# maxsonate/video-diffusion-nnx

Hardware: AMD Instinct MI355X
Metric: denoised frames/sec, 16fx64x64 1000-step DDPM (higher is better)
Workload: dtype bf16; 1 GPU; config_v2_2 (north-star shape): Unet3D dim=64 C=1, 16f x 64x64, DDPM T=1000 p_sample_loop (UNet forward + p_sample per step, hipGraph replay); value = n_gpus*B*F/(T*s_per_step); batch_per_gpu=64, parallelism=dp1 (independent samples, no collective), mfma_operands=bf16, storage=weights fp32 master, activations bf16, fp32 accumulate, process_group=none (single process)

## Files before the change

### video_diffusion_nnx_amd/csrc/conv_ws.hip

```cpp
#include "vdx_common.h"
#include "vdx_internal.h"
#include "vdx_glds.h"
#include <type_traits>

namespace vdx {

namespace {

__device__ __attribute__((aligned(16))) unsigned g_zero_page[4];

__device__ __forceinline__ int frag_off(int row, int key, int q) { return row * 128 + (((q ^ (key & 3)) | (key & 4)) << 4); }

constexpr int WS_SLAB = 128 * 128;
constexpr int WS_STORES = 16;

}

constexpr int WS_NS = 4;

template <int GEO> struct WsGeo {
    static constexpr bool WF = GEO != 0;
    static constexpr int S = WF ? GEO : 16;
    static constexpr int NP = WF ? 256 / (S * S) : 1;
    static constexpr int IW = 18;
    static constexpr int HPX = WF ? 257 : 18 * 18;
    static constexpr int NPIECE = HPX * 8;
    static constexpr int NU = (NPIECE + 511) / 512;
    static constexpr int NUMIN = NPIECE / 512;
    static constexpr int HBUF = HPX * 128;
};

template <int GEO, bool PRO>
__global__ __launch_bounds__(512, 2) void conv3x3_ws_kernel(const ConvArgs P, const int tiles_per_range, const int total_tiles, const int nct, const int pin) {
    using M = Mma<MODE_BF16>;
    using G = WsGeo<GEO>;
    constexpr bool WF = G::WF;
    constexpr int S = G::S, NP = G::NP, IW = G::IW, HPX = G::HPX, NPIECE = G::NPIECE, NU = G::NU, NUMIN = G::NUMIN, HBUF = G::HBUF;
    constexpr int NS = WS_NS;
    constexpr int WIN = 2;

    extern __shared__ __attribute__((aligned(16))) char smem[];
    char* ring = smem;
    char* halo = ring + NS * WS_SLAB;
    float* biasl = reinterpret_cast<float*>(halo + 2 * HBUF);
    float* coefA = biasl + 128;
    float* coefD = coefA + P.CinPad;
    float* gmean = coefD + P.CinPad;

    const unsigned ring_a = lds_addr(ring), halo_a = lds_addr(halo);
    const int tid = threadIdx.x, lane = tid & 63;
    const int wave = __builtin_amdgcn_readfirstlane(tid >> 6);
    const int r = lane & 15, q = lane >> 4;
    const int wc = wave & 1, wpx = wave >> 1;
    const int xcd = blockIdx.x & 7, slot = blockIdx.x >> 3;
    const int j = pin ? xcd % nct : slot % nct;
    const int range = pin ? slot * (8 / nct) + xcd / nct : (slot / nct) * 8 + xcd;
    const int t0 = range * tiles_per_range, t1 = min(t0 + tiles_per_range, total_tiles);
    if (t0 >= t1) return;
    const int tiles_x = WF ? 1 : P.W / 16, tiles_pf = WF ? 1 : tiles_x * (P.H / 16);
    const int nchunks = P.CinPad >> 6;
    const int Cin = P.C0 + P.C1;
    const int fpt = NP;
    const int tps = WF ? (P.F + NP - 1) / NP : 1;
    auto sample_of = [&](int t) { return WF ? t / tps : (t / tiles_pf) / P.F; };
    auto wf_pix0 = [&](int t) { const int b = t / tps, k = t - b * tps; return (unsigned)(b * P.F + k * NP) * (unsigned)(S * S); };
    auto wf_rows = [&](int t) { const int k = t % tps; return min(NP, P.F - k * NP) * (S * S); };

    unsigned wsrc[2];
#pragma unroll
    for (int v = 0; v < 2; ++v) {
        const int i2 = (v * 8 + wave) * 64 + lane, row = i2 >> 3, pos = i2 & 7;
        wsrc[v] = (unsigned)((j * 128 + row) * P.CinPad) * 2u + (unsigned)((pos ^ (row & 7)) << 4);
    }
    const size_t tap_stride = (size_t)P.Cout * P.CinPad * 2;
    const char* wbase = reinterpret_cast<const char*>(P.wp);
    auto piece = [&](int u, int l, int& row, int& chunk) -> bool {
        const int i = (u * 8 + wave) * 64 + l;
        row = i >> 3;
        const int key = WF ? row : row - ((row * 3641) >> 16) * IW;
        chunk = (i & 7) ^ (key & 7);
        return i < NPIECE;
    };
    auto opaque_lane = [&]() { int l = lane; asm volatile("" : "+v"(l)); return l; };
    const char* const zero_page = reinterpret_cast<const char*>(g_zero_page);
    constexpr int DYB = (WF ? S : IW) * 128;
    const int halo_o = NS * WS_SLAB;
    const int aoff = frag_off(wc * 64 + r, r, q);
    int b3[4][3], zs[3];
    int opix[4];
#pragma unroll
    for (int tn = 0; tn < 4; ++tn) {
        if (!WF) {
            const int py = wpx * 4 + tn, px = r;
            opix[tn] = py * P.W + px;
#pragma unroll
            for (int dx = 0; dx < 3; ++dx) b3[tn][dx] = halo_o + frag_off(py * IW + px + dx, px + dx, q);
        } else {
            const int p = wpx * 64 + tn * 16 + r;
            opix[tn] = p;
#pragma unroll
            for (int dx = 0; dx < 3; ++dx) b3[tn][dx] = halo_o + frag_off(p - S - 1 + dx, p - 1 + dx, q);
        }
    }
#pragma unroll
    for (int dy = 0; dy < 3; ++dy) zs[dy] = halo_o + 256 * 128 + (q << 4) - dy * DYB;
    auto tap_valid = [&](int tn, int dy, int dx) -> bool {
        const int p = wpx * 64 + tn * 16 + r, y = (p / S) % S + dy - 1, x = p % S + dx - 1;
        return y >= 0 && y < S && x >= 0 && x < S;
    };
    if (tid < 128) biasl[tid] = P.bias ? P.bias[j * 128 + tid] : 0.f;

    int pcc = 0, ptap = 0, pslot = 0;
    auto issue_w = [&]() {
        const char* src = wbase + (size_t)ptap * tap_stride + (size_t)(pcc << 7);
        const unsigned dst = __builtin_amdgcn_readfirstlane(ring_a + pslot * WS_SLAB + wave * 1024);
        glds16(src + wsrc[0], dst);
        glds16(src + wsrc[1], dst + 8 * 1024);
        if (++ptap == 9) { ptap = 0; if (++pcc == nchunks) pcc = 0; }
        if (++pslot == NS) pslot = 0;
    };
    unsigned okmask = 0;
    auto issue_halo = [&](int t, int cc, int buf) {
        const bool second = (cc << 6) >= P.C0;
        const char* xb = reinterpret_cast<const char*>(second ? P.x1 : P.x0);
        const int Cs = second ? P.C1 : P.C0, cb = (cc << 6) - (second ? P.C0 : 0);
        const unsigned dst = __builtin_amdgcn_readfirstlane(halo_a + buf * HBUF + wave * 1024);
        okmask = 0;
        const int l = opaque_lane();
        if (WF) {
            const unsigned pix0 = wf_pix0(t);
            const int nrows = wf_rows(t);
#pragma unroll
            for (int u = 0; u < NU; ++u) {
                int row, ch;
                if (piece(u, l, row, ch)) {
                    const bool ok = row < nrows;
                    const unsigned off = ((pix0 + row) * Cs + cb + (ch << 3)) * 2u;
                    const void* src = ok ? static_cast<const void*>(xb + off) : static_cast<const void*>(zero_page);
                    glds16(src, dst + u * 8 * 1024);
                    okmask |= ok ? (1u << u) : 0u;
                }
            }
        } else {
            const int f = t / tiles_pf, rem = t - f * tiles_pf, ty = rem / tiles_x, tx = rem - ty * tiles_x;
#pragma unroll
            for (int u = 0; u < NU; ++u) {
                int row, ch;
                if (piece(u, l, row, ch)) {
                    const int iy = (row * 3641) >> 16, ix = row - iy * IW;
                    const int gy = ty * 16 - 1 + iy, gx = tx * 16 - 1 + ix;
                    const bool ok = gy >= 0 && gy < P.H && gx >= 0 && gx < P.W;
                    const unsigned off = ((unsigned)((f * P.H + gy) * P.W + gx) * Cs + cb + (ch << 3)) * 2u;
                    const void* src = ok ? static_cast<const void*>(xb + off) : static_cast<const void*>(zero_page);
                    glds16(src, dst + u * 8 * 1024);
                    okmask |= ok ? (1u << u) : 0u;
                }
            }
        }
    };
    auto transform = [&](int u, int cc, int buf) {
        int row, ch;
        const int l = opaque_lane();
        if (!piece(u, l, row, ch) || !((okmask >> u) & 1u)) return;
        char* p = halo + buf * HBUF + ((u * 8 + wave) * 64 + l) * 16;
        const int c = (cc << 6) + (ch << 3);
#pragma unroll
        for (int h = 0; h < 2; ++h) {
            const uint2 v = *reinterpret_cast<const uint2*>(p + 8 * h);
            const float4 a = *reinterpret_cast<const float4*>(coefA + c + 4 * h);
            const float4 d = *reinterpret_cast<const float4*>(coefD + c + 4 * h);
            uint2 o;
            o.x = pack_bf16x2(silu_f(fmaf(__uint_as_float(v.x << 16), a.x, d.x)), silu_f(fmaf(__uint_as_float(v.x & 0xFFFF0000u), a.y, d.y)));
            o.y = pack_bf16x2(silu_f(fmaf(__uint_as_float(v.y << 16), a.z, d.z)), silu_f(fmaf(__uint_as_float(v.y & 0xFFFF0000u), a.w, d.w)));
            *reinterpret_cast<uint2*>(p + 8 * h) = o;
            asm volatile("" ::: "memory");
        }
    };
    auto make_coef = [&](int b) {
        gn_mean_rstd_wg(P.in_stats, b, P.groups, (double)P.F * P.H * P.W * (Cin / P.groups), gmean, tid, 512);
        __syncthreads();
        const int cpg = Cin / P.groups;
        for (int c = tid; c < Cin; c += 512) {
            const int g = c / cpg;
            const float m = gmean[2 * g], rs = gmean[2 * g + 1];
            const float ga = P.gamma[c], be = P.beta[c];
            float sc = 1.f, sh = 0.f;
            if (P.ss) { sc = P.ss[(size_t)b * P.ss_stride + c] + 1.f; sh = P.ss[(size_t)b * P.ss_stride + Cin + c]; }
            coefA[c] = rs * ga * sc;
            coefD[c] = (be - m * rs * ga) * sc + sh;
        }
        __syncthreads();
    };
    float st_s[4] = {0.f, 0.f, 0.f, 0.f}, st_q[4] = {0.f, 0.f, 0.f, 0.f};
    auto flush_stats = [&](int b) {
        if (!P.out_stats) return;
        const int cpg = P.Cout / P.out_groups;
#pragma unroll
        for (int tm = 0; tm < 4; ++tm) {
            const float s1 = reduce_q(reduce16(st_s[tm])), s2 = reduce_q(reduce16(st_q[tm]));
            st_s[tm] = 0.f; st_q[tm] = 0.f;
            if (lane == 0) {
                const int g = (j * 128 + wc * 64 + tm * 16) / cpg;
                double* dst = P.out_stats + (((size_t)b * GN_SLOTS + ((blockIdx.x + wave) % GN_SLOTS)) * P.out_groups + g) * 2;
                unsafeAtomicAdd(dst, (double)s1); unsafeAtomicAdd(dst + 1, (double)s2);
            }
        }
    };
    auto ldA1 = [&](int sl, int tm, int ks) -> uint4 {
        return *reinterpret_cast<const uint4*>(ring + sl * WS_SLAB + ((aoff + tm * 2048) ^ (ks * 64)));
    };
    auto ldB = [&](uint4 (&b)[4], int tap, int ks) {
        const int dy = tap / 3, dx = tap - 3 * dy;
#pragma unroll
        for (int tn = 0; tn < 4; ++tn) {
            int a = b3[tn][dx];
            if (WF) a = tap_valid(tn, dy, dx) ? a : zs[dy];
            b[tn] = *reinterpret_cast<const uint4*>(smem + ((a ^ (ks * 64)) + dy * DYB));
        }
    };
    auto flip_buffers = [&](int to_buf1) {
        const int d = to_buf1 ? HBUF : -HBUF;
#pragma unroll
        for (int tn = 0; tn < 4; ++tn)
#pragma unroll
            for (int dx = 0; dx < 3; ++dx) b3[tn][dx] += d;
#pragma unroll
        for (int dy = 0; dy < 3; ++dy) zs[dy] += d;
    };

    int bcoef = -1;
    const int b0 = sample_of(t0);
    if (PRO) { make_coef(b0); bcoef = b0; }
    issue_halo(t0, 0, 0);
#pragma unroll
    for (int k = 0; k < NS - 1; ++k) issue_w();
    wait_vm_lgkm0<0>();
    __builtin_amdgcn_s_barrier();
    if (PRO) {
#pragma unroll
        for (int u = 0; u < NU; ++u) transform(u, 0, 0);
        wait_vm_lgkm0<0>();
        __builtin_amdgcn_s_barrier();
    }

    int cslot = 0, hbuf = 0, bcur = b0;
    f32x4 acc[4][4];
    uint4 pb[4], pa;
    ldB(pb, 0, 0); pa = ldA1(0, 0, 0);
    auto run_chunk = [&](auto after_epi, int tnext, int ccnext, bool xform) {
        constexpr int EPI = decltype(after_epi)::value ? WS_STORES : 0;
#pragma unroll
        for (int tap = 0; tap < 9; ++tap) {
            if (tap == 0) wait_vm<WIN + EPI>();
            else if (tap == 1) wait_vm<WIN + NUMIN + EPI>();
            else wait_vm<WIN>();
            __builtin_amdgcn_s_barrier();
            if (tap == 0) issue_halo(tnext, ccnext, hbuf ^ 1);
            issue_w();
            const bool do_x = PRO && xform && tap >= 2 && tap - 2 < NU;
            if (do_x && wave < 4) {
                transform(tap - 2, ccnext, hbuf ^ 1);
                if (NU > 6 && tap == 7) transform(6, ccnext, hbuf ^ 1);
            }
#pragma unroll
            for (int tm = 0; tm < 4; ++tm) {
                const uint4 a = tm == 0 ? pa : ldA1(cslot, tm, 0);
#pragma unroll
                for (int tn = 0; tn < 4; ++tn) M::mma(acc[tm][tn], a, pb[tn]);
            }
            if (do_x && wave >= 4) {
                transform(tap - 2, ccnext, hbuf ^ 1);
                if (NU > 6 && tap == 7) transform(6, ccnext, hbuf ^ 1);
            }
            {
                uint4 b1[4];
                ldB(b1, tap, 1);
#pragma unroll
                for (int tm = 0; tm < 4; ++tm) {
                    const uint4 a = ldA1(cslot, tm, 1);
#pragma unroll
                    for (int tn = 0; tn < 4; ++tn) M::mma(acc[tm][tn], a, b1[tn]);
                }
            }
            const int nslot = (cslot + 1 == NS) ? 0 : cslot + 1;
            if (tap == 8) flip_buffers(hbuf ^ 1);
            ldB(pb, tap == 8 ? 0 : tap + 1, 0);
            pa = ldA1(nslot, 0, 0);
            cslot = nslot;
        }
        hbuf ^= 1;
    };

    bool after_epilogue = false;
    for (int t = t0; t < t1; ++t) {
#pragma unroll
        for (int tm = 0; tm < 4; ++tm)
#pragma unroll
            for (int tn = 0; tn < 4; ++tn) acc[tm][tn] = f32x4{0.f, 0.f, 0.f, 0.f};
        for (int cc = 0; cc < nchunks; ++cc) {
            const bool last = (cc + 1 == nchunks);
            const bool more = !last || (t + 1 < t1);
            const int tnext = last ? (t + 1 < t1 ? t + 1 : t) : t, ccnext = last ? 0 : cc + 1;
            if (PRO && more) {
                const int bn = sample_of(tnext);
                if (bn != bcoef) { make_coef(bn); bcoef = bn; }
            }
            if (after_epilogue) run_chunk(std::true_type{}, tnext, ccnext, more);
            else run_chunk(std::false_type{}, tnext, ccnext, more);
            after_epilogue = false;
        }
        {
            const int b = sample_of(t);
            if (b != bcur) { flush_stats(bcur); bcur = b; }
            size_t tile_pix;
            int nrows = 256;
            if (WF) { tile_pix = wf_pix0(t); nrows = wf_rows(t); }
            else { const int f = t / tiles_pf, rem = t - f * tiles_pf, ty = rem / tiles_x, tx = rem - ty * tiles_x;
                   tile_pix = ((size_t)f * P.H + (size_t)ty * 16) * P.W + (size_t)tx * 16; }
            const int cobase = j * 128 + wc * 64 + 4 * q;
#pragma unroll
            for (int tm = 0; tm < 4; ++tm) {
                float s = 0.f, ss = 0.f;
                const float4 bs = *reinterpret_cast<const float4*>(biasl + wc * 64 + tm * 16 + 4 * q);
#pragma unroll
                for (int tn = 0; tn < 4; ++tn) {
                    if (WF && opix[tn] >= nrows) continue;
                    const float4 v = make_float4(acc[tm][tn][0] + bs.x, acc[tm][tn][1] + bs.y, acc[tm][tn][2] + bs.z, acc[tm][tn][3] + bs.w);
                    const size_t e = (tile_pix + opix[tn]) * P.Cout + cobase + tm * 16;
                    if (P.y_bf16) *reinterpret_cast<uint2*>(reinterpret_cast<char*>(P.y) + e * 2) = make_uint2(pack_bf16x2(v.x, v.y), pack_bf16x2(v.z, v.w));
                    else *reinterpret_cast<float4*>(P.y + e) = v;
                    s += (v.x + v.y) + (v.z + v.w);
                    ss += (v.x * v.x + v.y * v.y) + (v.z * v.z + v.w * v.w);
                }
                st_s[tm] += s; st_q[tm] += ss;
            }
            after_epilogue = true;
        }
    }
    flush_stats(bcur);
    wait_vm_lgkm0<0>();
}

template <int GEO, int KIND, int BCO>
__global__ __launch_bounds__(512, 2) void conv4x4_ws_kernel(const ConvArgs P, const int tiles_per_range, const int total_vtiles, const int nct) {
    using M = Mma<MODE_BF16>;
    static_assert((GEO == 8 || GEO == 16 || GEO == 32) && (KIND == 1 || KIND == 2) && (BCO == 64 || BCO == 128), "geometry");
    constexpr bool BAND = GEO == 32;
    constexpr int S = GEO;
    constexpr int NP = BAND ? 1 : 256 / (S * S);
    constexpr int ZROW = BAND ? 320 : 256;
    constexpr int HPX = ZROW + 1, NPIECE = HPX * 8, NU = (NPIECE + 511) / 512, NUMIN = NPIECE / 512, HBUF = HPX * 128;
    constexpr int NS = WS_NS;
    constexpr int WIN = BCO / 64;
    constexpr int SLAB = BCO * 128;
    constexpr int TN = BCO == 128 ? 4 : 2;
    constexpr int STORES = 4 * TN;

    extern __shared__ __attribute__((aligned(16))) char smem[];
    char* ring = smem;
    char* halo = ring + NS * SLAB;
    float* biasl = reinterpret_cast<float*>(halo + 2 * HBUF);
    const unsigned ring_a = lds_addr(ring), halo_a = lds_addr(halo);
    const int tid = threadIdx.x, lane = tid & 63;
    const int wave = __builtin_amdgcn_readfirstlane(tid >> 6);
    const int r = lane & 15, q = lane >> 4;
    const int wc = BCO == 128 ? (wave & 1) : 0, wpx = BCO == 128 ? (wave >> 1) : wave;
    const int xcd = blockIdx.x & 7, slot = blockIdx.x >> 3;
    const int j = slot % nct;
    const int range = (slot / nct) * 8 + xcd;
    const int t0 = range * tiles_per_range, t1 = min(t0 + tiles_per_range, total_vtiles);
    if (t0 >= t1) return;
    const int C = P.C0;
    const int ncc = C >> 6;
    const int nchunks = KIND == 1 ? 4 * ncc : ncc;

    unsigned wsrc[WIN];
#pragma unroll
    for (int v = 0; v < WIN; ++v) {
        const int i2 = (v * 8 + wave) * 64 + lane, row = i2 >> 3, pos = i2 & 7;
        wsrc[v] = (unsigned)((j * BCO + row) * P.CinPad) * 2u + (unsigned)((pos ^ (row & 7)) << 4);
    }
    const size_t tap_stride = (size_t)P.Cout * P.CinPad * 2;
    const char* wbase = reinterpret_cast<const char*>(P.wp);
    auto piece = [&](int u, int l, int& row, int& chunk) -> bool {
        const int i = (u * 8 + wave) * 64 + l;
        row = i >> 3;
        chunk = (i & 7) ^ (row & 7);
        return i < NPIECE;
    };
    auto opaque_lane = [&]() { int l = lane; asm volatile("" : "+v"(l)); return l; };
    const char* const zero_page = reinterpret_cast<const char*>(g_zero_page);
    constexpr int DYB = S * 128;
    const int halo_o = NS * SLAB;
    const int aoff = frag_off(wc * 64 + r, r, q);
    int b3[TN][3], zs[3], opix[TN];
#pragma unroll
    for (int tn = 0; tn < TN; ++tn) {
        const int p = wpx * (TN * 16) + tn * 16 + r;
        if (KIND == 1) opix[tn] = p;
        else { const int fl = p / (S * S), y = (p / S) % S, x = p % S; opix[tn] = (fl * 2 * S + 2 * y) * 2 * S + 2 * x; }
#pragma unroll
        for (int dx = 0; dx < 3; ++dx) b3[tn][dx] = halo_o + frag_off(p - (BAND ? 0 : S) - 1 + dx, p - 1 + dx, q);
    }
#pragma unroll
    for (int dy = 0; dy < 3; ++dy) zs[dy] = halo_o + ZROW * 128 + (q << 4) - dy * DYB;
    auto tap_valid = [&](int tn, int dy, int dx) -> bool {
        const int p = wpx * (TN * 16) + tn * 16 + r, y = (p / S) % S + dy - 1, x = p % S + dx - 1;
        return (BAND || (y >= 0 && y < S)) && x >= 0 && x < S;
    };
    if (tid < BCO) biasl[tid] = P.bias ? P.bias[j * BCO + tid] : 0.f;

    int pph = t0 & 3, pcc = 0, ptap = 0, pslot = 0;
    auto issue_w = [&]() {
        const int ky = ptap >> 1, kx = ptap & 1;
        int widx, kofs;
        if (KIND == 1) { const int plane = pcc / ncc, cch = pcc - plane * ncc; widx = (1 - (plane >> 1) + 2 * ky) * 4 + (1 - (plane & 1) + 2 * kx); kofs = cch << 7; }
        else { widx = (2 * ky + (pph >> 1)) * 4 + (2 * kx + (pph & 1)); kofs = pcc << 7; }
        const char* src = wbase + (size_t)widx * tap_stride + (size_t)kofs;
        const unsigned dst = __builtin_amdgcn_readfirstlane(ring_a + pslot * SLAB + wave * 1024);
#pragma unroll
        for (int v = 0; v < WIN; ++v) glds16(src + wsrc[v], dst + v * 8 * 1024);
        if (++ptap == 4) { ptap = 0; if (++pcc == nchunks) { pcc = 0; pph = (pph + 1) & 3; } }
        if (++pslot == NS) pslot = 0;
    };
    auto issue_halo = [&](int vt, int cc, int buf) {
        const char* xb = reinterpret_cast<const char*>(P.x0);
        const unsigned dst = __builtin_amdgcn_readfirstlane(halo_a + buf * HBUF + wave * 1024);
        const int l = opaque_lane();
        const int plane = KIND == 1 ? cc / ncc : 0, cch = KIND == 1 ? cc - plane * ncc : cc;
        const int py = plane >> 1, px = plane & 1;
        const int tile = KIND == 1 ? vt : (vt >> 2);
#pragma unroll
        for (int u = 0; u < NU; ++u) {
            int row, ch;
            if (piece(u, l, row, ch)) {
                bool ok = row < ZROW;
                unsigned pix;
                if (BAND) {
                    const int f = tile >> 2, y = (tile & 3) * 8 + row / S - 1, x = row % S;
                    ok = ok && y >= 0 && y < S;
                    pix = KIND == 1 ? (unsigned)((f * 2 * S + 2 * y + py) * 2 * S + 2 * x + px) : (unsigned)((f * S + y) * S + x);
                } else if (KIND == 1) {
                    const int fl = row / (S * S), y = (row / S) % S, x = row % S;
                    pix = (unsigned)(((tile * NP + fl) * 2 * S + 2 * y + py) * 2 * S + 2 * x + px);
                } else pix = (unsigned)tile * 256u + row;
                const unsigned off = (pix * C + (cch << 6) + (ch << 3)) * 2u;
                const void* src = ok ? static_cast<const void*>(xb + off) : static_cast<const void*>(zero_page);
                glds16(src, dst + u * 8 * 1024);
            }
        }
    };
    auto ldA1 = [&](int sl, int tm, int ks) -> uint4 {
        return *reinterpret_cast<const uint4*>(ring + sl * SLAB + ((aoff + tm * 2048) ^ (ks * 64)));
    };
    auto flip_buffers = [&](int to_buf1) {
        const int d = to_buf1 ? HBUF : -HBUF;
#pragma unroll
        for (int tn = 0; tn < TN; ++tn)
#pragma unroll
            for (int dx = 0; dx < 3; ++dx) b3[tn][dx] += d;
#pragma unroll
        for (int dy = 0; dy < 3; ++dy) zs[dy] += d;
    };

    issue_halo(t0, 0, 0);
#pragma unroll
    for (int k = 0; k < NS - 1; ++k) issue_w();
    wait_vm_lgkm0<0>();
    __builtin_amdgcn_s_barrier();

    int cslot = 0, hbuf = 0;
    f32x4 acc[4][TN];
    auto run_chunk = [&](auto after_epi, auto ey_, auto ex_, int tnext, int ccnext) {
        constexpr int EPI = decltype(after_epi)::value ? STORES : 0;
        constexpr int EY = decltype(ey_)::value, EX = decltype(ex_)::value;
#pragma unroll
        for (int k = 0; k < 4; ++k) {
            constexpr int dummy = 0; (void)dummy;
            const int dy = EY + (k >> 1), dx = EX + (k & 1);
            if (k == 0) wait_vm<WIN + EPI>();
            else if (k == 1) wait_vm<WIN + NUMIN + EPI>();
            else wait_vm<WIN>();
            __builtin_amdgcn_s_barrier();
            if (k == 0) issue_halo(tnext, ccnext, hbuf ^ 1);
            issue_w();
#pragma unroll
            for (int ks = 0; ks < 2; ++ks) {
                uint4 b[TN];
#pragma unroll
                for (int tn = 0; tn < TN; ++tn) {
                    int a = b3[tn][dx];
                    a = tap_valid(tn, dy, dx) ? a : zs[dy];
                    b[tn] = *reinterpret_cast<const uint4*>(smem + ((a ^ (ks * 64)) + dy * DYB));
                }
#pragma unroll
                for (int tm = 0; tm < 4; ++tm) {
                    const uint4 a = ldA1(cslot, tm, ks);
#pragma unroll
                    for (int tn = 0; tn < TN; ++tn) M::mma(acc[tm][tn], a, b[tn]);
                }
            }
            if (k == 3) flip_buffers(hbuf ^ 1);
            cslot = (cslot + 1 == NS) ? 0 : cslot + 1;
        }
        hbuf ^= 1;
    };
    auto run_parity = [&](auto after_epi, int ey, int ex, int tnext, int ccnext) {
        using T0 = std::integral_constant<int, 0>; using T1 = std::integral_constant<int, 1>;
        if (ey == 0) { if (ex == 0) run_chunk(after_epi, T0{}, T0{}, tnext, ccnext); else run_chunk(after_epi, T0{}, T1{}, tnext, ccnext); }
        else { if (ex == 0) run_chunk(after_epi, T1{}, T0{}, tnext, ccnext); else run_chunk(after_epi, T1{}, T1{}, tnext, ccnext); }
    };

    bool after_epilogue = false;
    for (int t = t0; t < t1; ++t) {
#pragma unroll
        for (int tm = 0; tm < 4; ++tm)
#pragma unroll
            for (int tn = 0; tn < TN; ++tn) acc[tm][tn] = f32x4{0.f, 0.f, 0.f, 0.f};
        for (int cc = 0; cc < nchunks; ++cc) {
            const bool last = (cc + 1 == nchunks);
            const int tnext = last ? (t + 1 < t1 ? t + 1 : t) : t, ccnext = last ? 0 : cc + 1;
            int ey, ex;
            if (KIND == 1) { const int plane = cc / ncc; ey = 1 - (plane >> 1); ex = 1 - (plane & 1); }
            else { ey = (t & 3) >> 1; ex = t & 1; }
            if (after_epilogue) run_parity(std::true_type{}, ey, ex, tnext, ccnext);
            else run_parity(std::false_type{}, ey, ex, tnext, ccnext);
            after_epilogue = false;
        }
        {
            size_t tile_pix;
            if (KIND == 1) tile_pix = (size_t)t * 256;
            else tile_pix = (size_t)(t >> 2) * 1024 + (size_t)(((t & 3) >> 1) * 2 * S + (t & 1));
            const int cobase = j * BCO + wc * 64 + 4 * q;
#pragma unroll
            for (int tm = 0; tm < 4; ++tm) {
                const float4 bs = *reinterpret_cast<const float4*>(biasl + wc * 64 + tm * 16 + 4 * q);
#pragma unroll
                for (int tn = 0; tn < TN; ++tn) {
                    const float4 v = make_float4(acc[tm][tn][0] + bs.x, acc[tm][tn][1] + bs.y, acc[tm][tn][2] + bs.z, acc[tm][tn][3] + bs.w);
                    const size_t e = (tile_pix + opix[tn]) * P.Cout + cobase + tm * 16;
                    if (P.y_bf16) *reinterpret_cast<uint2*>(reinterpret_cast<char*>(P.y) + e * 2) = make_uint2(pack_bf16x2(v.x, v.y), pack_bf16x2(v.z, v.w));
                    else *reinterpret_cast<float4*>(P.y + e) = v;
                }
            }
            after_epilogue = true;
        }
    }
    wait_vm_lgkm0<0>();
}


static int ws_geo(const ConvArgs& a) {
    if (a.H == 8 && a.W == 8) return 8;
    if (a.H == 16 && a.W == 16) return 16;
    if (a.H % 16 == 0 && a.W % 16 == 0) return 0;
    return -1;
}

int conv3x3_ws_geo(const ConvArgs& a) { return ws_geo(a); }

static int ws4_geo(const ConvArgs& a) {
    const bool down = a.kind == 0 && a.kh == 4 && a.kw == 4 && a.stride == 2, up = a.kind == 1;
    if (!down && !up) return 0;
    const int s = down ? a.H / 2 : a.H;
    if (a.H != a.W || (down && (a.H % 2))) return 0;
    if (s == 32) return 32;
    if (s == 16) return 16;
    if (s == 8 && a.NF % 4 == 0) return 8;
    return 0;
}

bool conv4x4_ws_eligible(int mode, const ConvArgs& a) {
    if (mode != MODE_BF16 || a.res || a.pro || a.out_stats || a.C1 || !a.x0_bf16) return false;
    const int geo = ws4_geo(a);
    if (!geo) return false;
    if (a.C0 % 64 || (a.Cout % 128 && a.Cout != 64) || a.CinPad != a.C0) return false;
    const int nct = a.Cout == 64 ? 1 : a.Cout / 128;
    if (nct != 1 && nct != 2 && nct != 4 && nct != 8) return false;
    if (a.wrows != a.Cout || a.wrow0 != 0) return false;
    const long vtiles = (long)a.NF * geo * geo / 256 * (a.kind == 1 ? 4 : 1);
    if (vtiles * nct < 128) return false;
    if ((size_t)a.NF * a.H * a.W * (size_t)a.C0 * 2 >= 0xFFFF0000ull || (size_t)a.NF * 4 * geo * geo >= 0x7FFFFFFFull) return false;
    return true;
}

hipError_t launch_conv4x4_ws(const ConvArgs& a, hipStream_t st) {
    const int geo = ws4_geo(a), bco = a.Cout == 64 ? 64 : 128, nct = a.Cout / bco, up = a.kind == 1;
    const int total = (int)((long)a.NF * geo * geo / 256) * (up ? 4 : 1);
    const int cus = device_cus();
    const int unit = 8 * nct;
    int grid = std::max(unit, cus / unit * unit);
    grid = std::min(grid, (total * nct + unit - 1) / unit * unit);
    const int nranges = grid / nct;
    int tpr = (total + nranges - 1) / nranges;
    if (up) tpr = (tpr + 3) / 4 * 4;
    const size_t lds = (size_t)WS_NS * bco * 128 + 2 * (size_t)(geo == 32 ? 321 : 257) * 128 + 512;
    auto go = [&](auto kfn) -> hipError_t {
        if (hipError_t e = lds_opt_in(kfn, lds); e != hipSuccess) return e;
        hipLaunchKernelGGL(kfn, dim3(grid), dim3(512), lds, st, a, tpr, total, nct);
        return hipGetLastError();
    };
#define VDX_WS4(G_) do { if (bco == 64) return up ? go(conv4x4_ws_kernel<G_, 2, 64>) : go(conv4x4_ws_kernel<G_, 1, 64>);       \
                         return up ? go(conv4x4_ws_kernel<G_, 2, 128>) : go(conv4x4_ws_kernel<G_, 1, 128>); } while (0)
    if (geo == 8) VDX_WS4(8);
    if (geo == 16) VDX_WS4(16);
    VDX_WS4(32);
#undef VDX_WS4
}

bool conv3x3_ws_eligible(int mode, const ConvArgs& a) {
    if (mode != MODE_BF16 || a.kind != 0 || a.kh != 3 || a.kw != 3 || a.stride != 1 || a.res) return false;
    if (!a.x0_bf16 || (a.C1 && !a.x1_bf16)) return false;
    if (a.C0 % 64 || a.C1 % 64 || a.Cout % 128) return false;
    const int nct = a.Cout / 128;
    if (nct != 1 && nct != 2 && nct != 4 && nct != 8) return false;
    if (a.wrows != a.Cout || a.wrow0 != 0) return false;
    const int geo = ws_geo(a);
    if (geo < 0) return false;
    if (geo != 0 && (a.F <= 0 || a.NF % a.F)) return false;
    if (a.pro && (a.C1 || a.groups < 1 || a.groups > 32 || a.C0 % a.groups || a.C0 > 1024)) return false;
    if (a.out_stats && (a.out_groups < 1 || a.Cout % a.out_groups || (a.Cout / a.out_groups) % 16)) return false;
    const int npf = geo == 0 ? 1 : 256 / (a.H * a.W);
    const long tiles = geo == 0 ? (long)a.NF * (a.H / 16) * (a.W / 16) : (long)(a.NF / a.F) * ((a.F + npf - 1) / npf);
    if (tiles * nct < 128) return false;
    if ((size_t)a.NF * a.H * a.W * (size_t)std::max(a.C0, a.C1) * 2 >= 0xFFFF0000ull) return false;
    return true;
}

hipError_t launch_conv3x3_ws(const ConvArgs& a, hipStream_t st) {
    const int geo = ws_geo(a);
    const int nct = a.Cout / 128;
    const int npf = geo == 0 ? 1 : 256 / (a.H * a.W);
    const int total = geo == 0 ? a.NF * (a.H / 16) * (a.W / 16) : (a.NF / a.F) * ((a.F + npf - 1) / npf);
    const int cus = device_cus();
    const int unit = 8 * nct;
    int grid = std::max(unit, cus / unit * unit);
    grid = std::min(grid, (total * nct + unit - 1) / unit * unit);
    const int nranges = grid / nct;
    const int tpr = (total + nranges - 1) / nranges;
    const int HPX = geo == 0 ? 18 * 18 : 257;
    const size_t lds = (size_t)WS_NS * WS_SLAB + 2 * (size_t)HPX * 128 + 512 + (a.pro ? (size_t)a.CinPad * 8 + 256 : 0);
    if (lds > 160 * 1024) return hipErrorInvalidValue;
    auto go = [&](auto kfn) -> hipError_t {
        if (hipError_t e = lds_opt_in(kfn, lds); e != hipSuccess) return e;
#ifndef VDX_WS_PIN_MB
#define VDX_WS_PIN_MB 0
#endif
        const size_t wbytes = (size_t)9 * a.Cout * a.CinPad * 2;
        const int pin = (VDX_WS_PIN_MB > 0 && nct > 1 && wbytes > (size_t)VDX_WS_PIN_MB * 1024 * 1024) ? 1 : 0;
        hipLaunchKernelGGL(kfn, dim3(grid), dim3(512), lds, st, a, tpr, total, nct, pin);
        return hipGetLastError();
    };
    if (geo == 0) return a.pro ? go(conv3x3_ws_kernel<0, true>) : go(conv3x3_ws_kernel<0, false>);
    if (geo == 8) return a.pro ? go(conv3x3_ws_kernel<8, true>) : go(conv3x3_ws_kernel<8, false>);
    return a.pro ? go(conv3x3_ws_kernel<16, true>) : go(conv3x3_ws_kernel<16, false>);
}

}
```

Baseline: 49.95 frames/s.

## Slim register footprint of prologue conv3x3 WS kernel via LDS spills and recomputed addresses

For the GroupNorm+SiLU prologue variant, the kernel now recomputes per-tn B-fragment and output-pixel addresses from a single base instead of holding arrays in registers. It moves some per-wave GroupNorm output-stat accumulators into LDS and hoists the coefficient loads out of the transform. It also rewrites the mean/rstd reduction as a wave-level double shuffle reduction and changes the weight source offset. The goal is lower VGPR pressure so the prologue kernel can keep two workgroups per CU without spilling, at the cost of extra LDS traffic and a larger LDS allocation.

```diff
diff --git a/video_diffusion_nnx_amd/csrc/conv_ws.hip b/video_diffusion_nnx_amd/csrc/conv_ws.hip
--- a/video_diffusion_nnx_amd/csrc/conv_ws.hip
+++ b/video_diffusion_nnx_amd/csrc/conv_ws.hip
@@ -38,6 +38,9 @@
     constexpr int S = G::S, NP = G::NP, IW = G::IW, HPX = G::HPX, NPIECE = G::NPIECE, NU = G::NU, NUMIN = G::NUMIN, HBUF = G::HBUF;
     constexpr int NS = WS_NS;
     constexpr int WIN = 2;
+    constexpr bool SLIM = PRO;
+    constexpr int STL = SLIM ? (WF ? 4 : 1) : 0;
+    constexpr int TNB = (WF ? 16 : IW) * 128;
 
     extern __shared__ __attribute__((aligned(16))) char smem[];
     char* ring = smem;
@@ -46,6 +49,7 @@
     float* coefA = biasl + 128;
     float* coefD = coefA + P.CinPad;
     float* gmean = coefD + P.CinPad;
+    float* stl = gmean + 64;
 
     const unsigned ring_a = lds_addr(ring), halo_a = lds_addr(halo);
     const int tid = threadIdx.x, lane = tid & 63;
@@ -115,7 +119,8 @@
         const char* src = wbase + (size_t)ptap * tap_stride + (size_t)(pcc << 7);
         const unsigned dst = __builtin_amdgcn_readfirstlane(ring_a + pslot * WS_SLAB + wave * 1024);
         glds16(src + wsrc[0], dst);
-        glds16(src + wsrc[1], dst + 8 * 1024);
+        if (SLIM) glds16(src + (size_t)P.CinPad * 128 + wsrc[0], dst + 8 * 1024);
+        else glds16(src + wsrc[1], dst + 8 * 1024);
         if (++ptap == 9) { ptap = 0; if (++pcc == nchunks) pcc = 0; }
         if (++pslot == NS) pslot = 0;
     };
@@ -158,17 +163,25 @@
             }
         }
     };
-    auto transform = [&](int u, int cc, int buf) {
-        int row, ch;
+    float4 cfa[2], cfd[2];
+    auto load_coef = [&](int cc) {
+        const int c = (cc << 6) + ((opaque_lane() & 7) << 3);
+#pragma unroll
+        for (int h = 0; h < 2; ++h) {
+            cfa[h] = *reinterpret_cast<const float4*>(coefA + c + 4 * h);
+            cfd[h] = *reinterpret_cast<const float4*>(coefD + c + 4 * h);
+        }
+    };
+    auto transform = [&](int u, int t, int buf) {
+        int row, pos;
         const int l = opaque_lane();
-        if (!piece(u, l, row, ch) || !((okmask >> u) & 1u)) return;
-        char* p = halo + buf * HBUF + ((u * 8 + wave) * 64 + l) * 16;
-        const int c = (cc << 6) + (ch << 3);
+        if (!piece(u, l, row, pos)) return;
+        if (WF ? row >= wf_rows(t) : !((okmask >> u) & 1u)) return;
+        char* p = halo + buf * HBUF + row * 128 + (pos << 4);
 #pragma unroll
         for (int h = 0; h < 2; ++h) {
             const uint2 v = *reinterpret_cast<const uint2*>(p + 8 * h);
-            const float4 a = *reinterpret_cast<const float4*>(coefA + c + 4 * h);
-            const float4 d = *reinterpret_cast<const float4*>(coefD + c + 4 * h);
+            const float4 a = cfa[h], d = cfd[h];
             uint2 o;
             o.x = pack_bf16x2(silu_f(fmaf(__uint_as_float(v.x << 16), a.x, d.x)), silu_f(fmaf(__uint_as_float(v.x & 0xFFFF0000u), a.y, d.y)));
             o.y = pack_bf16x2(silu_f(fmaf(__uint_as_float(v.y << 16), a.z, d.z)), silu_f(fmaf(__uint_as_float(v.y & 0xFFFF0000u), a.w, d.w)));
@@ -177,7 +190,29 @@
         }
     };
     auto make_coef = [&](int b) {
-        gn_mean_rstd_wg(P.in_stats, b, P.groups, (double)P.F * P.H * P.W * (Cin / P.groups), gmean, tid, 512);
+        const int tid = wave * 64 + opaque_lane();
+        {
+            const double count = (double)P.F * P.H * P.W * (Cin / P.groups);
+            auto xor_d = [&](double v, int o) {
+                const int idx = ((tid & 63) ^ o) << 2;
+                const int lo = __builtin_amdgcn_ds_bpermute(idx, __double2loint(v)), hi = __builtin_amdgcn_ds_bpermute(idx, __double2hiint(v));
+                return __hiloint2double(hi, lo);
+            };
+            for (int t = tid; t < P.groups * GN_SLOTS; t += 512) {
+                const int g = t >> 5, slot = t & 31;
+                const double2 v = *reinterpret_cast<const double2*>(P.in_stats + (((size_t)b * GN_SLOTS + slot) * P.groups + g) * 2);
+                double s = v.x, ss = v.y;
+#pragma unroll
+                for (int o = 16; o >= 1; o >>= 1) { s += xor_d(s, o); ss += xor_d(ss, o); }
+                if (slot == 0) {
+                    const double m = s / count;
+                    double var = ss / count - m * m;
+                    if (var < 0.0) var = 0.0;
+                    gmean[2 * g] = (float)m;
+                    gmean[2 * g + 1] = (float)(1.0 / sqrt(var + (double)NORM_EPS));
+                }
+            }
+        }
         __syncthreads();
         const int cpg = Cin / P.groups;
         for (int c = tid; c < Cin; c += 512) {
@@ -192,13 +227,21 @@
         __syncthreads();
     };
     float st_s[4] = {0.f, 0.f, 0.f, 0.f}, st_q[4] = {0.f, 0.f, 0.f, 0.f};
+    if (STL > 0) {
+#pragma unroll
+        for (int k = 0; k < 2 * STL; ++k) stl[k * 512 + tid] = 0.f;
+    }
     auto flush_stats = [&](int b) {
         if (!P.out_stats) return;
         const int cpg = P.Cout / P.out_groups;
 #pragma unroll
         for (int tm = 0; tm < 4; ++tm) {
-            const float s1 = reduce_q(reduce16(st_s[tm])), s2 = reduce_q(reduce16(st_q[tm]));
-            st_s[tm] = 0.f; st_q[tm] = 0.f;
+            float ps, pq;
+            if (STL > 0 && tm >= 4 - STL) {
+                float* sl = stl + (tm - (4 - STL)) * 1024 + wave * 64 + opaque_lane();
+                ps = sl[0]; pq = sl[512]; sl[0] = 0.f; sl[512] = 0.f;
+            } else { ps = st_s[tm]; pq = st_q[tm]; st_s[tm] = 0.f; st_q[tm] = 0.f; }
+            const float s1 = reduce_q(reduce16(ps)), s2 = reduce_q(reduce16(pq));
             if (lane == 0) {
                 const int g = (j * 128 + wc * 64 + tm * 16) / cpg;
                 double* dst = P.out_stats + (((size_t)b * GN_SLOTS + ((blockIdx.x + wave) % GN_SLOTS)) * P.out_groups + g) * 2;
@@ -211,21 +254,29 @@
     };
     auto ldB = [&](uint4 (&b)[4], int tap, int ks) {
         const int dy = tap / 3, dx = tap - 3 * dy;
+        int bs = 0, zr = 0;
+        if (SLIM) { bs = b3[0][dx]; zr = zs[0]; asm volatile("" : "+v"(bs)); if (WF) asm volatile("" : "+v"(zr)); }
 #pragma unroll
         for (int tn = 0; tn < 4; ++tn) {
-            int a = b3[tn][dx];
-            if (WF) a = tap_valid(tn, dy, dx) ? a : zs[dy];
-            b[tn] = *reinterpret_cast<const uint4*>(smem + ((a ^ (ks * 64)) + dy * DYB));
+            if (SLIM) {
+                int a = bs;
+                if (WF) a = tap_valid(tn, dy, dx) ? a : zr - (dy * DYB + tn * TNB);
+                b[tn] = *reinterpret_cast<const uint4*>(smem + ((a ^ (ks * 64)) + (dy * DYB + tn * TNB)));
+            } else {
+                int a = b3[tn][dx];
+                if (WF) a = tap_valid(tn, dy, dx) ? a : zs[dy];
+                b[tn] = *reinterpret_cast<const uint4*>(smem + ((a ^ (ks * 64)) + dy * DYB));
+            }
         }
     };
     auto flip_buffers = [&](int to_buf1) {
         const int d = to_buf1 ? HBUF : -HBUF;
 #pragma unroll
-        for (int tn = 0; tn < 4; ++tn)
+        for (int tn = 0; tn < (SLIM ? 1 : 4); ++tn)
 #pragma unroll
             for (int dx = 0; dx < 3; ++dx) b3[tn][dx] += d;
 #pragma unroll
-        for (int dy = 0; dy < 3; ++dy) zs[dy] += d;
+        for (int dy = 0; dy < (SLIM ? 1 : 3); ++dy) zs[dy] += d;
     };
 
     int bcoef = -1;
@@ -237,8 +288,9 @@
     wait_vm_lgkm0<0>();
     __builtin_amdgcn_s_barrier();
     if (PRO) {
-#pragma unroll
-        for (int u = 0; u < NU; ++u) transform(u, 0, 0);
+        load_coef(0);
+#pragma unroll
+        for (int u = 0; u < NU; ++u) transform(u, t0, 0);
         wait_vm_lgkm0<0>();
         __builtin_amdgcn_s_barrier();
     }
@@ -258,9 +310,10 @@
             if (tap == 0) issue_halo(tnext, ccnext, hbuf ^ 1);
             issue_w();
             const bool do_x = PRO && xform && tap >= 2 && tap - 2 < NU;
+            if (PRO && xform && tap == 2) load_coef(ccnext);
             if (do_x && wave < 4) {
-                transform(tap - 2, ccnext, hbuf ^ 1);
-                if (NU > 6 && tap == 7) transform(6, ccnext, hbuf ^ 1);
+                transform(tap - 2, tnext, hbuf ^ 1);
+                if (NU > 6 && tap == 7) transform(6, tnext, hbuf ^ 1);
             }
 #pragma unroll
             for (int tm = 0; tm < 4; ++tm) {
@@ -269,8 +322,8 @@
                 for (int tn = 0; tn < 4; ++tn) M::mma(acc[tm][tn], a, pb[tn]);
             }
             if (do_x && wave >= 4) {
-                transform(tap - 2, ccnext, hbuf ^ 1);
-                if (NU > 6 && tap == 7) transform(6, ccnext, hbuf ^ 1);
+                transform(tap - 2, tnext, hbuf ^ 1);
+                if (NU > 6 && tap == 7) transform(6, tnext, hbuf ^ 1);
             }
             {
                 uint4 b1[4];
@@ -317,22 +370,29 @@
             if (WF) { tile_pix = wf_pix0(t); nrows = wf_rows(t); }
             else { const int f = t / tiles_pf, rem = t - f * tiles_pf, ty = rem / tiles_x, tx = rem - ty * tiles_x;
                    tile_pix = ((size_t)f * P.H + (size_t)ty * 16) * P.W + (size_t)tx * 16; }
-            const int cobase = j * 128 + wc * 64 + 4 * q;
+            const int le = SLIM ? opaque_lane() : lane;
+            const int qe = SLIM ? le >> 4 : q;
+            const int op0 = SLIM ? (WF ? wpx * 64 + (le & 15) : wpx * 4 * P.W + (le & 15)) : 0;
+            const int cobase = j * 128 + wc * 64 + 4 * qe;
 #pragma unroll
             for (int tm = 0; tm < 4; ++tm) {
                 float s = 0.f, ss = 0.f;
-                const float4 bs = *reinterpret_cast<const float4*>(biasl + wc * 64 + tm * 16 + 4 * q);
+                const float4 bs = *reinterpret_cast<const float4*>(biasl + wc * 64 + tm * 16 + 4 * qe);
 #pragma unroll
                 for (int tn = 0; tn < 4; ++tn) {
-                    if (WF && opix[tn] >= nrows) continue;
+                    const int op = SLIM ? op0 + tn * (WF ? 16 : P.W) : opix[tn];
+                    if (WF && op >= nrows) continue;
                     const float4 v = make_float4(acc[tm][tn][0] + bs.x, acc[tm][tn][1] + bs.y, acc[tm][tn][2] + bs.z, acc[tm][tn][3] + bs.w);
-                    const size_t e = (tile_pix + opix[tn]) * P.Cout + cobase + tm * 16;
+                    const size_t e = (tile_pix + op) * P.Cout + cobase + tm * 16;
                     if (P.y_bf16) *reinterpret_cast<uint2*>(reinterpret_cast<char*>(P.y) + e * 2) = make_uint2(pack_bf16x2(v.x, v.y), pack_bf16x2(v.z, v.w));
                     else *reinterpret_cast<float4*>(P.y + e) = v;
                     s += (v.x + v.y) + (v.z + v.w);
                     ss += (v.x * v.x + v.y * v.y) + (v.z * v.z + v.w * v.w);
                 }
-                st_s[tm] += s; st_q[tm] += ss;
+                if (STL > 0 && tm >= 4 - STL) {
+                    float* sl = stl + (tm - (4 - STL)) * 1024 + wave * 64 + le;
+                    sl[0] += s; sl[512] += ss;
+                } else { st_s[tm] += s; st_q[tm] += ss; }
             }
             after_epilogue = true;
         }
@@ -639,7 +699,7 @@
     const int nranges = grid / nct;
     const int tpr = (total + nranges - 1) / nranges;
     const int HPX = geo == 0 ? 18 * 18 : 257;
-    const size_t lds = (size_t)WS_NS * WS_SLAB + 2 * (size_t)HPX * 128 + 512 + (a.pro ? (size_t)a.CinPad * 8 + 256 : 0);
+    const size_t lds = (size_t)WS_NS * WS_SLAB + 2 * (size_t)HPX * 128 + 512 + (a.pro ? (size_t)a.CinPad * 8 + 256 + (geo == 0 ? 1 : 4) * 4096 : 0);
     if (lds > 160 * 1024) return hipErrorInvalidValue;
     auto go = [&](auto kfn) -> hipError_t {
         if (hipError_t e = lds_opt_in(kfn, lds); e != hipSuccess) return e;
```

Measured after the change: 49.92 frames/s (median of 4 runs). Within noise of the previous version (-0.1%).
